# wvu-irl/flope

Hardware: AMD Instinct MI355X
Metric: poses_per_sec (higher is better)
Workload: dtype f16; 1 GPU; PoseResNet (ResNet-18 trunk + fp32 head) forward + special Procrustes + pose assembly, batch 256 x 224x224x3 16-bit NHWC crops resident in HBM per GPU (BASELINE configs[1]); one RCCL all-gather of the poses per run when N>1 (configs[3]); batch_per_gpu=256, global_batch=256, crop=224, parallelism=dp1, weights=synthetic_state_dict(seed 0), eval-mode BN folded

## Files before the change

### flope_amd/csrc/engine.hip

```cpp
#include "../../include/flope_amd.h"
#include "common.h"
#include "host_pack.h"

#include <math.h>
#include <stdio.h>
#include <stdlib.h>
#include <string.h>

#include <map>
#include <string>
#include <vector>

extern "C" int flope_conv_mfma_init();
extern "C" int flope_conv_mfma_launch(const ConvP* p, int dtype, int cfg, int patch, int nbuf, size_t lds, void* stream);
extern "C" int flope_stem_init();
extern "C" int flope_stem_launch(const StemP* p, int dtype, size_t lds, void* stream);
extern "C" int flope_maxpool_launch(const PoolP* p, int dtype, void* stream);
extern "C" int flope_avgpool_launch(const void* in, float* out, int B, int h, int w, int C, int dtype, void* stream);
extern "C" int flope_fc1_launch(const float* feat, const float* W1, const float* W1p, const float* b1, float* hidden, int B, int K, int N, void* stream);
extern "C" int flope_fc2_procrustes_launch(const float* hidden, const float* W2, const float* b2, float* r9, float* R, int B, int K, const float* xyz, int nullify, float* Rt, void* stream);
extern "C" int flope_fc2_procrustes_k4_launch(const float* hidden, const float* W2, const float* b2, float* r9, float* R, int B, int K, const float* xyz, int nullify, float* Rt, void* stream);
extern "C" int flope_prep_input_launch(const void* x, int in_format, int B, int H, int W, void* out, int Hip, int Wip, int dtype, void* stream);
extern "C" int flope_read_stage_launch(const void* in, float* out, int B, int C, int h, int w, int dtype, void* stream);
extern "C" int flope_naive_conv_launch(const NaiveConvP* p, void* stream);
extern "C" int flope_conv_stag_init();
extern "C" int flope_conv_gstag_init();
extern "C" int flope_conv_w4_init();
extern "C" int flope_conv_r4_init();
extern "C" int flope_conv_r4_ok(const ConvP* p);
extern "C" int flope_conv_r4_launch(const ConvP* p, int dtype, int grid_blocks, void* stream);
extern "C" int flope_conv_s1r_init();
extern "C" int flope_conv_s1r_ok(const ConvP* p);
extern "C" int flope_conv_s1r_launch(const ConvP* p, const void* w, int dtype, int grid, void* stream);
extern "C" int flope_conv_s2r_init();
extern "C" int flope_conv_s2r_ok(const ConvP* p);
extern "C" int flope_conv_s2r_launch(const ConvP* p, const void* w, int dtype, int grid, void* stream);
extern "C" int flope_conv_w4_launch(const ConvP* p, int dtype, int grid_blocks, int mt, void* stream);
extern "C" size_t flope_conv_w4_lds(int pt, int mt, int dsf, int pers);
extern "C" int flope_conv_gstag_launch(const ConvP* p, int dtype, void* stream);
extern "C" int flope_conv_stag_launch(const ConvP* p, int dtype, int grid_blocks, size_t lds, void* stream);
extern "C" int flope_conv_split_finalize_launch(const ConvP* p, int dtype, void* stream);
extern "C" int flope_stem_pool_init();
extern "C" int flope_stem_pool_r_blocks_per_cu();
#ifdef FLOPE_STAG_DBG
extern "C" void flope_stem_pool_set_dbg(void* ptr);
#endif
// ... 12 lines not shown
constexpr size_t kDbgRegion = 1 << 20;
constexpr size_t kBufSlack = 1 << 20;

struct Conv {
  std::string name, bn;
  int cin = 0, cout = 0, k = 0, stride = 1;
  int in_buf = -1, out_buf = -1, res_buf = -1;
  int hin = 0, win = 0, hout = 0, wout = 0;
  int relu = 0;
  int cfg = 0, patch = 0, nbuf = 2, per_image = 0, tiles_per_image = 0, mtiles = 0, ntiles = 0, rows_max = 0;
  size_t lds = 0;
  void* w_packed = nullptr;
  void* w_stag = nullptr;
  void* w_s2r = nullptr;
  void* w_s1r = nullptr;
  int stag = 0, stag_patch_bytes = 0, nseg = 1; size_t stag_lds = 0;
  int w4_patch[9] = {0};
  float* w_naive = nullptr;
  float* bias = nullptr;
  int folded = 0, ds_conv = -1;
  void* w_ds_stag = nullptr;
  void* w_ds_s1r = nullptr;
  float* bias_fused = nullptr;
  mutable std::string last_kernel, last_detail;
};

struct Buf { void* ptr = nullptr; size_t bytes = 0; int C = 0, h = 0, w = 0; };

}

struct flope_engine {
  int device = 0, H = 0, W = 0, maxB = 0, dtype = 0, bod = 2048;
  int esz = 2;
  int sHip = 0, sWip = 0, Hs = 0, Ws = 0, stem_tiles = 0, stem_rows = 0;
  size_t stem_lds = 0;
  void* stem_in = nullptr; size_t stem_in_bytes = 0;
  int* stem_q = nullptr;
  void* stem_w = nullptr; void* stem_w2 = nullptr; float* stem_w_naive = nullptr; float* stem_bias = nullptr;
  std::vector<Buf> bufs;
  std::vector<Conv> convs;
  int stage_buf[10];
  int final_buf = -1;
  float *feat = nullptr, *hidden = nullptr, *W1 = nullptr, *W1p = nullptr, *b1 = nullptr, *W2 = nullptr, *b2 = nullptr;
  float* r9_scratch = nullptr;
  bool weights_loaded = false;
  int opt_patch = 1, opt_bm256 = 1, opt_profile = 0, opt_nbuf = 2, opt_dbg = 0, opt_ldspad = 0, opt_fuse_stem = 1, opt_streams = 2, opt_persist = 0, num_cus = 256, opt_stag = 3, cur_slices = 1, plan_slices = 1, cur_batch = 1, opt_rows_grid = 0, opt_split = 0, opt_dsfuse = 1, opt_ksplit = 1, opt_fc1_packed = 1, opt_gstag = 1, opt_rowseg = 1, opt_stem_persist = 1, opt_skew = 1, opt_reslds = 1, opt_prio = 0, opt_r4 = 1, opt_w4cw = 4, opt_w4cwf = 0, opt_fc2_k4 = 1, opt_w4mt = 0, opt_w4mtlo = 0, opt_lag = 20, opt_w4 = 1, opt_stem_r = 1, opt_s2r = 1, opt_s2r_grid = 0, opt_s1r = 1;
  float* split_ws = nullptr; size_t split_ws_bytes = 0;
  hipStream_t side[4] = {nullptr, nullptr, nullptr, nullptr};
  hipEvent_t ev_fork = nullptr, ev_join[4] = {nullptr, nullptr, nullptr, nullptr};
  std::vector<hipEvent_t> ev;
  int ev_n = 0;
  std::vector<int> ev_slice;
  int mark_slice = 0;
  int last_batch = 0;
  bool last_fused = false;
  std::string err;
};

namespace {

int fail(flope_engine* e, int code, const std::string& msg) {
// ... 218 lines not shown
extern "C" const char* flope_version(void) { return "flope_amd 0.1 (gfx950; mfma_f32_16x16x32 bf16/f16; fp32 head)"; }

extern "C" int flope_engine_geometry(flope_handle h, int* max_batch, int* dtype, int* height, int* width, int* device_id) {
  if (!h) return FLOPE_EINVAL;
  if (max_batch) *max_batch = h->maxB;
  if (dtype) *dtype = h->dtype;
  if (height) *height = h->H;
  if (width) *width = h->W;
  if (device_id) *device_id = h->device;
  return FLOPE_OK;
}

extern "C" const char* flope_last_error(flope_handle h) { return h ? h->err.c_str() : g_last_error.c_str(); }

static int rebuild_plan(flope_engine* e) {
  for (Conv& c : e->convs) { plan_conv(e, c); c.folded = 0; c.ds_conv = -1; }
  if (e->opt_dsfuse && e->dtype != FLOPE_DT_F32)
    for (size_t i = 0; i + 1 < e->convs.size(); ++i) {
      Conv& cd = e->convs[i];
      Conv& c2 = e->convs[i + 1];
      if (cd.k == 1 && c2.k == 3 && c2.res_buf == cd.out_buf && c2.stag == 1 && c2.cout >= 128 && c2.stag_patch_bytes >= 4 &&
          c2.stag_patch_bytes != 7 && cd.cin % 64 == 0 && cd.stride == 2) {
        cd.folded = 1;
        c2.ds_conv = (int)i;
      }
    }
  return 0;
}

extern "C" int flope_create(int device_id, int height, int width, int max_batch, int dtype, int backbone_out_dim,
                            flope_handle* out) {
// ... 24 lines not shown
  {
    hipDeviceProp_t prop;
    CREATE_TRY(hipGetDeviceProperties(&prop, device_id));
    e->num_cus = prop.multiProcessorCount > 0 ? prop.multiProcessorCount : 256;
  }
  if (dtype != FLOPE_DT_F32) {
    int s = flope_conv_mfma_init();
    if (s == 0) s = flope_stem_init();
    if (s == 0) s = flope_stem_pool_init();
    if (s == 0) s = flope_conv_stag_init();
    if (s == 0) s = flope_conv_gstag_init();
    if (s == 0) s = flope_conv_w4_init();
    if (s == 0) s = flope_conv_r4_init();
    if (s == 0) s = flope_conv_s2r_init();
    if (s == 0) s = flope_conv_s1r_init();
    if (s != 0) { int rc = fail(nullptr, FLOPE_EHIP, std::string("kernel attribute setup: ") + hipGetErrorString((hipError_t)s)); flope_destroy(e); return rc; }
  }
  const size_t B = (size_t)max_batch;
  e->sHip = height + 6; e->sWip = (width + 8 + 1) & ~1;
  e->Hs = out_dim(height, 7, 2, 3); e->Ws = out_dim(width, 7, 2, 3);
  e->stem_in_bytes = B * e->sHip * e->sWip * 4 * e->esz;
  CREATE_TRY(hipMalloc(&e->stem_in, e->stem_in_bytes));
  CREATE_TRY(hipMemset(e->stem_in, 0, e->stem_in_bytes));
  {
    const int HoWo = e->Hs * e->Ws;
    e->stem_tiles = (HoWo + 255) / 256;
    int span = 1;
    for (int t = 0; t < e->stem_tiles; ++t) {
      const int m0 = t * 256, me = std::min(m0 + 256, HoWo);
      span = std::max(span, (me - 1) / e->Ws - m0 / e->Ws + 1);
// ... 62 lines not shown
  e->ev.resize(4 * (e->convs.size() + 8) + 2);
  e->ev_slice.assign(e->ev.size(), 0);
  for (hipEvent_t& ev : e->ev) CREATE_TRY(hipEventCreate(&ev));
  CREATE_TRY(hipDeviceSynchronize());
#undef CREATE_TRY
  rebuild_plan(e);
  *out = e;
  return FLOPE_OK;
}

extern "C" int flope_destroy(flope_handle e) {
  if (!e) return FLOPE_OK;
  hipSetDevice(e->device);
  hipDeviceSynchronize();
  for (Buf& b : e->bufs) if (b.ptr) hipFree(b.ptr);
  for (Conv& c : e->convs) { if (c.w_packed) hipFree(c.w_packed); if (c.w_stag) hipFree(c.w_stag); if (c.w_s2r) hipFree(c.w_s2r); if (c.w_s1r) hipFree(c.w_s1r); if (c.w_naive) hipFree(c.w_naive); if (c.bias) hipFree(c.bias); if (c.w_ds_stag) hipFree(c.w_ds_stag); if (c.w_ds_s1r) hipFree(c.w_ds_s1r); if (c.bias_fused) hipFree(c.bias_fused); }
  void* singles[] = {e->stem_in, e->stem_q, e->stem_w, e->stem_w2, e->stem_w_naive, e->stem_bias, e->feat, e->hidden, e->W1, e->W1p, e->b1, e->W2, e->b2, e->r9_scratch, e->split_ws};
  for (void* p : singles) if (p) hipFree(p);
  for (hipEvent_t ev : e->ev) hipEventDestroy(ev);
  for (int i = 0; i < 4; ++i) { if (e->side[i]) hipStreamDestroy(e->side[i]); if (e->ev_join[i]) hipEventDestroy(e->ev_join[i]); }
  if (e->ev_fork) hipEventDestroy(e->ev_fork);
  delete e;
  return FLOPE_OK;
}

extern "C" int flope_debug_read_ws(flope_handle e, void* dst_host, size_t offset, size_t bytes) {
  if (!e || !dst_host) return fail(e, FLOPE_EINVAL, "flope_debug_read_ws: NULL argument");
  if (!e->split_ws || offset + bytes > e->split_ws_bytes) return fail(e, FLOPE_EINVAL, "flope_debug_read_ws: out of range");
  HIP_TRY(e, hipSetDevice(e->device));
  HIP_TRY(e, hipDeviceSynchronize());
  HIP_TRY(e, hipMemcpy(dst_host, (const char*)e->split_ws + offset, bytes, hipMemcpyDeviceToHost));
// ... 6 lines not shown
  if (!strcmp(name, "patch")) { prev = e->opt_patch; e->opt_patch = value != 0; }
  else if (!strcmp(name, "bm256")) { prev = e->opt_bm256; e->opt_bm256 = value != 0; }
  else if (!strcmp(name, "persist")) { prev = e->opt_persist; e->opt_persist = value != 0; return prev; }
  else if (!strcmp(name, "rows_grid")) { prev = e->opt_rows_grid; e->opt_rows_grid = value < 0 ? -1 : value; return prev; }
  else if (!strcmp(name, "split")) { prev = e->opt_split; e->opt_split = value < 0 ? 0 : value; return prev; }
  else if (!strcmp(name, "fc1_packed")) { prev = e->opt_fc1_packed; e->opt_fc1_packed = value != 0; return prev; }
  else if (!strcmp(name, "w4mtlo")) { prev = e->opt_w4mtlo; e->opt_w4mtlo = value <= 0 ? 0 : (value < 5 ? 5 : (value > 8 ? 8 : value)); return prev; }
  else if (!strcmp(name, "lag")) { prev = e->opt_lag; e->opt_lag = value < 0 ? 0 : (value > 500 ? 500 : value); return prev; }
  else if (!strcmp(name, "w4mt")) { prev = e->opt_w4mt; e->opt_w4mt = (value >= 5 && value <= 8) ? value : 0; return prev; }
  else if (!strcmp(name, "fc2_k4")) { prev = e->opt_fc2_k4; e->opt_fc2_k4 = value != 0; return prev; }
  else if (!strcmp(name, "ksplit")) { prev = e->opt_ksplit; e->opt_ksplit = value < 0 ? 0 : (value > 2 ? 2 : value); return prev; }
  else if (!strcmp(name, "stem_r")) { prev = e->opt_stem_r; e->opt_stem_r = value != 0; return prev; }
  else if (!strcmp(name, "stem_persist")) { prev = e->opt_stem_persist; e->opt_stem_persist = value < 0 ? 0 : (value > 2 ? 2 : value); return prev; }
  else if (!strcmp(name, "rowseg")) { prev = e->opt_rowseg; e->opt_rowseg = value != 0; }
  else if (!strcmp(name, "skew")) { prev = e->opt_skew; e->opt_skew = value != 0; }
  else if (!strcmp(name, "r4")) { prev = e->opt_r4; e->opt_r4 = value != 0; return prev; }
  else if (!strcmp(name, "s1r")) { prev = e->opt_s1r; e->opt_s1r = value != 0; return prev; }
  else if (!strcmp(name, "s2r_grid")) { prev = e->opt_s2r_grid; e->opt_s2r_grid = value; return prev; }
  else if (!strcmp(name, "s2r")) { prev = e->opt_s2r; e->opt_s2r = value != 0; return prev; }
  else if (!strcmp(name, "w4")) { prev = e->opt_w4; e->opt_w4 = value != 0; return prev; }
  else if (!strcmp(name, "w4cw")) { prev = e->opt_w4cw; e->opt_w4cw = value < 0 ? 0 : (value > 64 ? 64 : value); return prev; }
  else if (!strcmp(name, "w4cwf")) { prev = e->opt_w4cwf; e->opt_w4cwf = value & 3; return prev; }
  else if (!strcmp(name, "prio")) { prev = e->opt_prio; e->opt_prio = value < 0 ? 0 : (value > 2 ? 2 : value); return prev; }
  else if (!strcmp(name, "reslds")) { prev = e->opt_reslds; e->opt_reslds = value != 0; return prev; }
  else if (!strcmp(name, "gstag")) { prev = e->opt_gstag; e->opt_gstag = value < 0 ? 0 : (value > 2 ? 2 : value); }
  else if (!strcmp(name, "dsfuse")) { prev = e->opt_dsfuse; e->opt_dsfuse = value != 0; }
  else if (!strcmp(name, "stag")) { prev = e->opt_stag; e->opt_stag = value < 0 ? 0 : (value > 3 ? 3 : value); }
  else if (!strcmp(name, "streams")) { prev = e->opt_streams; e->opt_streams = value < 1 ? 1 : (value > 4 ? 4 : value); return prev; }
  else if (!strcmp(name, "fuse_stem")) { prev = e->opt_fuse_stem; e->opt_fuse_stem = value != 0; return prev; }
  else if (!strcmp(name, "ldspad")) { prev = e->opt_ldspad; e->opt_ldspad = value; return prev; }
  else if (!strcmp(name, "dbg")) { prev = e->opt_dbg; e->opt_dbg = value; return prev; }
// ... 24 lines not shown
  if ((rc = fold(e, ts, "base.conv1", "base.bn1", 64, 3, 7, &wf, &bf)) != 0) return rc;
  if ((rc = upload(e, bf, (void**)&e->stem_bias)) != 0) return rc;
  if (e->dtype == FLOPE_DT_F32) { if ((rc = upload(e, naive_layout(wf, 64, 3, 7), (void**)&e->stem_w_naive)) != 0) return rc; }
  else {
    if ((rc = upload(e, pack_stem(wf, e->dtype), &e->stem_w)) != 0) return rc;
    if ((rc = upload(e, pack_stem_frag(wf, e->dtype), &e->stem_w2)) != 0) return rc;
  }
  for (Conv& c : e->convs) {
    if ((rc = fold(e, ts, c.name, c.bn, c.cout, c.cin, c.k, &wf, &bf)) != 0) return rc;
    if ((rc = upload(e, bf, (void**)&c.bias)) != 0) return rc;
    if (e->dtype == FLOPE_DT_F32) { if ((rc = upload(e, naive_layout(wf, c.cout, c.cin, c.k), (void**)&c.w_naive)) != 0) return rc; }
    else {
      if ((rc = upload(e, pack_conv(wf, c.cout, c.cin, c.k, e->dtype), &c.w_packed)) != 0) return rc;
      if (c.k == 3 && c.cin % 64 == 0 && (rc = upload(e, pack_conv32(wf, c.cout, c.cin, e->dtype), &c.w_stag)) != 0) return rc;
      if (c.k == 3 && c.stride == 1 && c.cin == 128 && c.cout == 128 && (rc = upload(e, pack_s1r(wf, c.cin, e->dtype), &c.w_s1r)) != 0) return rc;
      if (c.k == 3 && c.stride == 2 && c.cin == 64 && c.cout == 128 && (rc = upload(e, pack_s2r(wf, c.cout, c.cin, e->dtype), &c.w_s2r)) != 0) return rc;
      if (c.k == 1 && c.stride == 2 && c.cin == 64 && c.cout == 128 && (rc = upload(e, pack_s1r_ds(wf, c.cin, e->dtype), &c.w_ds_s1r)) != 0) return rc;
      if (c.k == 1 && c.cout >= 128 && c.cin % 64 == 0 && (rc = upload(e, pack_conv32_1x1(wf, c.cout, c.cin, e->dtype), &c.w_ds_stag)) != 0) return rc;
    }
    host_bias.push_back(bf);
  }
  for (size_t i = 0; i + 1 < e->convs.size(); ++i)
    if (e->convs[i].k == 1 && e->convs[i + 1].res_buf == e->convs[i].out_buf) {
      std::vector<float> sum = host_bias[i + 1];
      for (size_t j = 0; j < sum.size(); ++j) sum[j] += host_bias[i][j];
      if ((rc = upload(e, sum, (void**)&e->convs[i + 1].bias_fused)) != 0) return rc;
    }
  const float* w1 = ts.get(e, "base.fc.0.weight", {e->bod, 512}, &rc); if (!w1) return rc;
  const float* b1 = ts.get(e, "base.fc.0.bias", {e->bod}, &rc); if (!b1) return rc;
  const float* w2 = ts.get(e, "fc_rot.weight", {9, e->bod}, &rc); if (!w2) return rc;
// ... 58 lines not shown
      K_TRY(e, "stem (fp32)", flope_naive_conv_launch(&p, stream));
    } else {
      StemP p; memset(&p, 0, sizeof(p));
      p.in = stem_in; p.out = bs.ptr; p.w = e->stem_w; p.bias = e->stem_bias;
      p.B = batch; p.Hip = e->sHip; p.Wip = e->sWip; p.Ho = e->Hs; p.Wo = e->Ws;
      p.tiles_per_image = e->stem_tiles; p.patch_rows_max = e->stem_rows;
      SMARK();
      K_TRY(e, "stem", flope_stem_launch(&p, dt, e->stem_lds, stream));
    }
    PoolP pp; pp.in = bs.ptr; pp.out = bp.ptr; pp.B = batch; pp.Hip = bs.h + 2; pp.Wip = bs.w + 2; pp.C = 64; pp.Ho = bp.h; pp.Wo = bp.w;
    SMARK();
    K_TRY(e, "maxpool", flope_maxpool_launch(&pp, dt, stream));
  }
  for (const Conv& c : e->convs) {
    if (c.folded) continue;
    if (dt == FLOPE_DT_F32) {
      NaiveConvP p; memset(&p, 0, sizeof(p));
      p.in = (const float*)vb[c.in_buf].ptr; p.out = (float*)vb[c.out_buf].ptr;
      p.res = c.res_buf >= 0 ? (const float*)vb[c.res_buf].ptr : nullptr;
      p.w = c.w_naive; p.bias = c.bias;
      p.B = batch; p.Hip = c.hin + 2; p.Wip = c.win + 2; p.Cin_stored = c.cin; p.Cin = c.cin; p.Ho = c.hout; p.Wo = c.wout;
      p.Hop = c.hout + 2; p.Wop = c.wout + 2; p.Cout = c.cout; p.KH = c.k; p.KW = c.k; p.stride = c.stride;
      p.in_off = c.k == 3 ? 0 : 1; p.relu = c.relu;
      SMARK();
      K_TRY(e, c.name.c_str(), flope_naive_conv_launch(&p, stream));
    } else if (c.stag == 3) {
      ConvP p; conv_params(e, vb, c, batch, &p);
      p.w = c.w_stag; p.per_image = 0; p.mtiles = (p.M + 255) / 256; p.ntiles = c.cout / 128; p.total_tiles = p.mtiles * p.ntiles;
      SMARK();
      c.last_kernel = "conv_gstag_kernel<256x128,s2>"; c.last_detail.clear();
// ... 250 lines not shown
}

extern "C" double flope_forward_flops(flope_handle e, int batch) {
  if (!e) return 0.0;
  double macs = (double)e->Hs * e->Ws * 64 * 147;
  for (const Conv& c : e->convs) macs += (double)c.hout * c.wout * c.cout * c.cin * c.k * c.k;
  macs += 512.0 * e->bod + 9.0 * e->bod;
  return 2.0 * macs * batch;
}

static int head_launches(const flope_engine* e) { return (e->opt_fuse_stem && e->dtype != FLOPE_DT_F32) ? 1 : 3; }
static int tail_launches(const flope_engine*) { return 3; }
extern "C" int flope_forward_launches(flope_handle e) {
  if (!e) return 0;
  int n = (int)e->convs.size() + tail_launches(e) + head_launches(e);
  for (const Conv& c : e->convs) n -= c.folded;
  return n;
}

extern "C" int flope_profile_read(flope_handle e, float* ms_out, int cap) {
  if (!e || !ms_out) return fail(e, FLOPE_EINVAL, "flope_profile_read: NULL argument");
  if (e->opt_profile != 1 || e->ev_n < 2) return fail(e, FLOPE_ESTATE, "flope_profile_read: no forward with option profile = 1 (profile = 2 records a time line: flope_profile_timeline)");
  HIP_TRY(e, hipEventSynchronize(e->ev[e->ev_n - 1]));
  const int n = std::min(cap, e->ev_n - 1);
  for (int i = 0; i < n; ++i) HIP_TRY(e, hipEventElapsedTime(&ms_out[i], e->ev[i], e->ev[i + 1]));
  return n;
}

extern "C" int flope_profile_timeline(flope_handle e, float* ms_out, int* slice_out, int cap) {
  if (!e || !ms_out || !slice_out) return fail(e, FLOPE_EINVAL, "flope_profile_timeline: NULL argument");
  if (e->opt_profile != 2 || e->ev_n < 2) return fail(e, FLOPE_ESTATE, "flope_profile_timeline: no forward with option profile = 2");
  HIP_TRY(e, hipSetDevice(e->device));
  HIP_TRY(e, hipDeviceSynchronize());
  const int n = std::min(cap, e->ev_n);
  for (int i = 0; i < n; ++i) {
    ms_out[i] = 0.f;
    if (i > 0) HIP_TRY(e, hipEventElapsedTime(&ms_out[i], e->ev[0], e->ev[i]));
    slice_out[i] = e->ev_slice[i];
  }
  return n;
}

extern "C" int flope_launch_info(flope_handle e, int idx, int batch, char* name, int name_cap, double* flops) {
  if (!e || !name || name_cap < 1 || !flops) return fail(e, FLOPE_EINVAL, "flope_launch_info: NULL argument");
  std::vector<int> live;
  for (size_t i = 0; i < e->convs.size(); ++i) if (!e->convs[i].folded) live.push_back((int)i);
  const int nc = (int)live.size();
  const int nh = head_launches(e);
  if (idx < 0 || idx >= nc + tail_launches(e) + nh) return fail(e, FLOPE_EINVAL, "flope_launch_info: bad index");
  const bool f32 = e->dtype == FLOPE_DT_F32;
  std::string s; double f = 0.0;
  if (nh == 1) {
    if (idx == 0) { s = "input+stem+maxpool|stem_pool_kernel"; f = 2.0 * e->Hs * e->Ws * 64 * 147; }
  } else {
    if (idx == 0) s = "prep_input|prep_input_kernel";
    else if (idx == 1) { s = f32 ? "stem|naive_conv_kernel" : "stem|stem_mfma_kernel"; f = 2.0 * e->Hs * e->Ws * 64 * 147; }
    else if (idx == 2) s = "maxpool|maxpool_kernel";
  }
  idx += 3 - nh;
  if (idx < 3) {  }
  else if (idx < 3 + nc) {
    const Conv& c = e->convs[live[idx - 3]];
    int BM, BN; tile_dims(c.cfg, &BM, &BN);
    char k[96];
    if (f32) snprintf(k, sizeof k, "naive_conv_kernel");
    else if (c.stag == 3) snprintf(k, sizeof k, "conv_gstag_kernel<256x128,s2>");
    else if (e->opt_s1r && c.w_s1r && (c.ds_conv < 0 || e->convs[c.ds_conv].w_ds_s1r) && c.stag == 1 && c.wout == 28 && c.hout % 4 == 0) snprintf(k, sizeof k, "conv_s1r_kernel<4rows x28>");
    else if (w4_eligible(e, c)) snprintf(k, sizeof k, "conv_w4_kernel<256x128>");
    else if (c.stag == 2 && e->opt_r4 && c.nseg <= 1 && c.cin == 64 && c.cout == 64 && c.wout == 56 && c.hout % 8 == 0) snprintf(k, sizeof k, "conv_r4_kernel<8rows x56>");
    else if (c.stag) snprintf(k, sizeof k, c.stag == 2 ? "conv_stag_kernel<8rows x64>" : (c.cout == 64 ? "conv_stag_kernel<512x64>" : "conv_stag_kernel<256x128>"));
    else if (e->opt_s2r && c.w_s2r && c.wout == 28 && c.hout % 4 == 0) snprintf(k, sizeof k, "conv_s2r_kernel<4rows x28>");
    else snprintf(k, sizeof k, "conv_mfma_kernel<%dx%d,%s,ring%d>", BM, BN, c.patch ? "patch" : "gather", c.nbuf);
    if (!f32 && e->last_batch > 0 && !c.last_kernel.empty()) snprintf(k, sizeof k, "%s", c.last_kernel.c_str());
    s = c.name + ((!f32 && e->last_batch > 0) ? c.last_detail : std::string()) + "|" + k;
    f = 2.0 * c.hout * c.wout * c.cout * c.cin * c.k * c.k;
    if (c.ds_conv >= 0) {
      const Conv& cd = e->convs[c.ds_conv];
      s = c.name + "+shortcut" + ((!f32 && e->last_batch > 0) ? c.last_detail : std::string()) + "|" + k;
      f += 2.0 * cd.hout * cd.wout * cd.cout * cd.cin;
    }
  } else if (idx == 3 + nc) s = "avgpool|avgpool_kernel";
  else if (idx == 4 + nc) { s = "fc1|fc1_kernel"; f = 2.0 * 512 * e->bod; }
  else { s = "fc_rot+procrustes|fc2_procrustes_kernel"; f = 2.0 * 9 * e->bod; }
  snprintf(name, name_cap, "%s", s.c_str());
  *flops = f * batch;
  return FLOPE_OK;
}

extern "C" int flope_describe_plan(flope_handle e, char* buf, int buflen) {
  if (!e || !buf || buflen < 1) return FLOPE_EINVAL;
  std::string s;
  char line[256];
  snprintf(line, sizeof line, "stem: tiles/img=%d rows=%d lds=%zu\n", e->stem_tiles, e->stem_rows, e->stem_lds);
  s += line;
  for (const Conv& c : e->convs) {
    if (c.stag == 3) { snprintf(line, sizeof line, "%s: 3x3 s2 %d->%d out %dx%d conv_gstag 256x128 (gathered tiles) lds=147456\n", c.name.c_str(), c.cin, c.cout, c.hout, c.wout); s += line; continue; }
    if (c.folded) { snprintf(line, sizeof line, "%s: 1x1 s2 %d->%d out %dx%d folded into the next conv (conv_stag DSF)\n", c.name.c_str(), c.cin, c.cout, c.hout, c.wout); s += line; continue; }
    if (c.stag && c.ds_conv >= 0) { snprintf(line, sizeof line, "%s: 3x3 s1 %d->%d out %dx%d %s 256x128 patch_rounds=%d lds=%zu, shortcut folded in (+%d K)\n", c.name.c_str(), c.cin, c.cout, c.hout, c.wout, w4_eligible(e, c) ? "conv_w4" : "conv_stag", c.stag_patch_bytes, c.stag_lds, e->convs[c.ds_conv].cin); s += line; continue; }
    if (c.stag == 2 && c.nseg > 1) { snprintf(line, sizeof line, "%s: 3x3 s1 %d->%d out %dx%d conv_stag 8-row bands x %d column segments of 64 patch_rounds=%d lds=%zu\n", c.name.c_str(), c.cin, c.cout, c.hout, c.wout, c.nseg, c.stag_patch_bytes, c.stag_lds); s += line; continue; }
    if (c.stag == 1 && w4_eligible(e, c)) { snprintf(line, sizeof line, "%s: 3x3 s1 %d->%d out %dx%d conv_w4 256x128 patch_rounds=%d lds=%zu\n", c.name.c_str(), c.cin, c.cout, c.hout, c.wout, c.stag_patch_bytes, flope_conv_w4_lds(c.stag_patch_bytes, 8, 0, 0)); s += line; continue; }
    if (c.stag) { snprintf(line, sizeof line, c.stag == 2 ? "%s: 3x3 s1 %d->%d out %dx%d conv_stag 8-row bands x 64 patch_rounds=%d lds=%zu\n" : "%s: 3x3 s1 %d->%d out %dx%d conv_stag 256x128 patch_rounds=%d lds=%zu\n", c.name.c_str(), c.cin, c.cout, c.hout, c.wout, c.stag_patch_bytes, c.stag_lds); s += line; continue; }
    snprintf(line, sizeof line, "%s: %dx%d s%d %d->%d out %dx%d cfg=%d patch=%d ring=%d per_image=%d rows=%d lds=%zu\n", c.name.c_str(),
             c.k, c.k, c.stride, c.cin, c.cout, c.hout, c.wout, c.cfg, c.patch, c.nbuf, c.per_image, c.rows_max, c.lds);
    s += line;
  }
  snprintf(buf, buflen, "%s", s.c_str());
  return FLOPE_OK;
}
```

### flope_amd/csrc/host_pack.h

```cpp
#pragma once
#include <stdint.h>
#include <string.h>
#include <vector>

#define FLOPE_DT_BF16_ 0

namespace flope_host {

inline void fastdiv_magic(unsigned d, unsigned* mg, unsigned* sh) {
  unsigned l = 0;
  while ((1ull << l) < d) ++l;
  const unsigned long long num = 1ull << (31 + l);
  *mg = (unsigned)((num + d - 1) / d);
  *sh = 31 + l;
}

inline uint16_t f32_to_bf16(float f) {
  uint32_t u; memcpy(&u, &f, 4);
  if ((u & 0x7fffffffu) > 0x7f800000u) return (uint16_t)((u >> 16) | 0x0040u);
  u += 0x7fffu + ((u >> 16) & 1u);
  return (uint16_t)(u >> 16);
}

inline uint16_t f32_to_f16(float f) {
// ... 152 lines not shown
}

inline std::vector<uint16_t> pack_s1r_ds(const std::vector<float>& wf, int cin, int dtype) {
  std::vector<uint16_t> out((size_t)4 * 2 * 2 * 64 * 8);
  for (int cg = 0; cg < 4; ++cg)
    for (int kh = 0; kh < 2; ++kh)
      for (int ct = 0; ct < 2; ++ct)
        for (int lane = 0; lane < 64; ++lane)
          for (int j = 0; j < 8; ++j) {
            const int i = lane & 15, co = 32 * cg + 8 * (i >> 2) + 4 * ct + (i & 3), ci = 32 * kh + 8 * (lane >> 4) + j;
            out[((((size_t)cg * 2 + kh) * 2 + ct) * 64 + lane) * 8 + j] = cvt16(wf[(size_t)co * cin + ci], dtype);
          }
  return out;
}

inline std::vector<float> naive_layout(const std::vector<float>& wf, int cout, int cin, int k) {
  std::vector<float> out((size_t)cout * cin * k * k);
  for (int co = 0; co < cout; ++co)
    for (int ci = 0; ci < cin; ++ci)
      for (int ky = 0; ky < k; ++ky)
        for (int kx = 0; kx < k; ++kx)
          out[(((size_t)ky * k + kx) * cin + ci) * cout + co] = wf[(((size_t)co * cin + ci) * k + ky) * k + kx];
  return out;
}


inline std::vector<float> pack_fc1(const float* W1, int N, int K) {
  std::vector<float> out((size_t)N * K);
  const int KB = K / 32;
  for (int t = 0; t < N / 16; ++t)
// ... 11 lines not shown
```

Baseline: 262,700 poses/s.

## Fuse layer1 basic-block conv pairs into one kernel with LDS intermediate

Adds a conv_l1f kernel that runs both 3x3 64->64 convolutions of a layer1 basic block in one launch. Producer waves compute conv1 rows into an LDS ring while consumer waves compute conv2 plus the residual from the staged input. Each image is split into row-pair segments chosen by a cost heuristic. This removes the HBM round trip of the intermediate activation and one launch per block, in exchange for more LDS, a single block per CU, and halo recomputation at segment edges.

```diff
diff --git a/flope_amd/csrc/conv_l1f.hip b/flope_amd/csrc/conv_l1f.hip
--- /dev/null
+++ b/flope_amd/csrc/conv_l1f.hip
@@ -0,0 +1,281 @@
+#include "common.h"
+#include <type_traits>
+
+namespace {
+
+#pragma clang diagnostic push
+#pragma clang diagnostic ignored "-Winline-asm"
+__device__ __forceinline__ void l1f_glds16(const char* gptr, unsigned lds_addr) {
+  asm volatile("s_mov_b32 m0, %1\n\ts_nop 0\n\tglobal_load_lds_dwordx4 %0, off" ::"v"(gptr), "s"(lds_addr) : "memory", "m0");
+}
+#pragma clang diagnostic pop
+
+__device__ __forceinline__ int l1f_tile_px(int c) { return c < 4 ? 2 * c : (c < 12 ? 2 * (c - 4) + 1 : 2 * (c - 8)); }
+
+constexpr int kWo = 56, kPairs = 28, kRowB = 64 * 64, kNin = 10, kNim = 8, kStep = 18;
+constexpr int kInPlane = kNin * kRowB;
+constexpr int kImOff = 2 * kInPlane;
+constexpr int kImPlane = kNim * kRowB;
+constexpr int kLds = kImOff + 2 * kImPlane;
+
+struct L1fP {
+  const void* in;
+  void* out;
+  const float* bias1;
+  const float* bias2;
+  int B, Hip, Wip;
+  int nseg;
+  int relu1, relu2;
+};
+
+#define L1F_BARRIER()                                                                                          \
+  do {                                                                                                         \
+    __builtin_amdgcn_sched_barrier(0);                                                                         \
+    asm volatile("" ::: "memory");                                                                             \
+    __builtin_amdgcn_s_barrier();                                                                              \
+    asm volatile("" ::: "memory");                                                                             \
+    __builtin_amdgcn_sched_barrier(0);                                                                         \
+  } while (0)
+
+template <typename T, int ROLE, int P0, int NP>
+__device__ __forceinline__ void l1f_walk(const L1fP& p, const u32x4* __restrict__ wpk, char* smem, int wave, int lane) {
+  typedef typename Elem<T>::frag frag;
+  const int tid = wave * 64 + lane, g = lane >> 4, r16 = lane & 15, cg = wave & 1;
+  const int pcol = l1f_tile_px(r16);
+  const bool t3row = pcol >= 8;
+  int cst[9];
+#pragma unroll
+  for (int t = 0; t < 9; ++t) {
+    const int dy = t / 3, c = pcol + t % 3;
+    cst[t] = c * 64 + ((g ^ ((2 * (dy & 1) + (c >> 2)) & 3)) << 4);
+  }
+
+  const u32x4* const wl = wpk + (size_t)cg * kStep * 2 * 64 + lane;
+  frag wres[kStep][2];
+  f32x4 b4[2];
+#pragma unroll
+  for (int s = 0; s < kStep; ++s)
+#pragma unroll
+    for (int ct = 0; ct < 2; ++ct) wres[s][ct] = __builtin_bit_cast(frag, wl[(s * 2 + ct) * 64]);
+  const float* const bias = ROLE ? p.bias2 : p.bias1;
+#pragma unroll
+  for (int ct = 0; ct < 2; ++ct) b4[ct] = *(const f32x4*)(bias + 32 * cg + 8 * g + 4 * ct);
+
+  const int drow = wave & 1, dplane = (wave >> 1) & 1;
+  int dsrc[4];
+#pragma unroll
+  for (int j = 0; j < 4; ++j) {
+    const int px = 16 * j + (lane >> 2);
+    dsrc[j] = (drow * p.Wip + min(px, p.Wip - 1)) * 128 + dplane * 64 + (((lane & 3) ^ ((2 * drow + (px >> 2)) & 3)) << 4);
+  }
+  auto dma_pair = [&](int img, int rp) {
+    const char* const src = (const char*)p.in + ((size_t)img * p.Hip + rp) * p.Wip * 128;
+    const unsigned dst = (unsigned)(dplane * kInPlane + ((rp % kNin) + drow) * kRowB);
+#pragma unroll
+    for (int j = 0; j < 4; ++j)
+      l1f_glds16(src + dsrc[j], (unsigned)__builtin_amdgcn_readfirstlane((int)(dst + j * 1024 + (unsigned)(size_t)(__attribute__((address_space(3))) char*)smem)));
+  };
+
+#pragma unroll
+  for (int i = 0; i < 2 * kImPlane / (512 * 16); ++i) *(u32x4*)(smem + kImOff + (i * 512 + tid) * 16) = u32x4{0u, 0u, 0u, 0u};
+#pragma unroll
+  for (int s = 0; s < kStep; ++s)
+#pragma unroll
+    for (int ct = 0; ct < 2; ++ct) asm volatile("" : "+v"(wres[s][ct]));
+#pragma unroll
+  for (int ct = 0; ct < 2; ++ct) asm volatile("" : "+v"(b4[ct]));
+
+  int ooff[NP];
+#pragma unroll
+  for (int i = 0; i < NP; ++i) {
+    const int k = (P0 + i) * 16 + pcol, row = k >= kWo ? 1 : 0, col = k - row * kWo;
+    ooff[i] = ((row * p.Wip + col + 1) * 64 + 32 * cg + 8 * g) * 2;
+  }
+
+  auto vbase = [&](const int (&sb)[4], const int (&v3)[3], int grp, int t) -> int {
+    const int dy = t / 3;
+    int a = (grp == 0 ? sb[dy] : (grp == 1 ? v3[dy] : sb[dy + 1] + 512)) + cst[t];
+    asm volatile("" : "+v"(a));
+    return a;
+  };
+  auto tgrp = [](int pt) { return pt < 3 ? 0 : (pt == 3 ? 1 : 2); };
+  auto toff = [](int pt) { return pt < 3 ? pt * 1024 : (pt == 3 ? 0 : (pt - 4) * 1024); };
+  constexpr bool kG0 = P0 == 0, kG1 = P0 == 0 && NP == 4, kG2 = P0 + NP > 4;
+  auto step_bases = [&](const int (&sb)[4], const int (&v3)[3], int t, int (&va)[3]) {
+    if (kG0) va[0] = vbase(sb, v3, 0, t);
+    if (kG1) va[1] = vbase(sb, v3, 1, t);
+    if (kG2) va[2] = vbase(sb, v3, 2, t);
+  };
+  auto faddr = [&](const int (&va)[3], int pt, int hc, int plane_b) -> char* { return smem + va[tgrp(pt)] + toff(pt) + hc * plane_b; };
+  auto ring = [&](int off, int n, int R, int (&sb)[4], int (&v3)[3]) {
+#pragma unroll
+    for (int lr = 0; lr < 4; ++lr) sb[lr] = off + ((R + lr) % n) * kRowB;
+#pragma unroll
+    for (int dy = 0; dy < 3; ++dy) v3[dy] = t3row ? sb[dy + 1] - 512 : sb[dy] + 3072;
+  };
+
+  const int G = gridDim.x, total = p.B * p.nseg, L = kPairs / p.nseg;
+  for (int item = blockIdx.x; item < total; item += G) {
+    const int img = item / p.nseg, s0 = (item - img * p.nseg) * L, s1 = s0 + L;
+    const int p0 = max(s0 - 1, 0), p1 = min(s1, kPairs - 1);
+    if (s0 == 0) {
+      *(u32x4*)(smem + kImOff + (tid >> 8) * kImPlane + (tid & 255) * 16) = u32x4{0u, 0u, 0u, 0u};
+    }
+    if constexpr (ROLE == 0) {
+      dma_pair(img, 2 * p0);
+      dma_pair(img, 2 * p0 + 2);
+      asm volatile("s_waitcnt vmcnt(0)" ::: "memory");
+    }
+    asm volatile("s_waitcnt lgkmcnt(0)" ::: "memory");
+    L1F_BARRIER();
+    for (int q = p0; q <= s1 + 1; ++q) {
+      int sb[4], v3[3];
+      if constexpr (ROLE == 0) {
+        if (q + 1 <= p1) dma_pair(img, 2 * q + 4);
+        int wb[4], w3[3];
+        ring(kImOff, kNim, 2 * q, wb, w3);
+        f32x4 acc[NP][2];
+        if (q <= p1) {
+          ring(0, kNin, 2 * q, sb, v3);
+          frag xf[2][NP];
+          int va[3] = {0, 0, 0};
+          step_bases(sb, v3, 0, va);
+#pragma unroll
+          for (int pt = 0; pt < NP; ++pt) xf[0][pt] = *(const frag*)faddr(va, P0 + pt, 0, kInPlane);
+          __builtin_amdgcn_sched_barrier(0);
+#pragma unroll
+          for (int s = 0; s < kStep; ++s) {
+            if (s + 1 < kStep) step_bases(sb, v3, (s + 1) % 9, va);
+#pragma unroll
+            for (int pt = 0; pt < NP; ++pt) {
+#pragma unroll
+              for (int ct = 0; ct < 2; ++ct) acc[pt][ct] = Elem<T>::mfma(wres[s][ct], xf[s & 1][pt], s == 0 ? b4[ct] : acc[pt][ct]);
+              if (s + 1 < kStep) xf[(s + 1) & 1][pt] = *(const frag*)faddr(va, P0 + pt, (s + 1) / 9, kInPlane);
+              __builtin_amdgcn_sched_group_barrier(0x008, 2, 0);
+              if (s + 1 < kStep) __builtin_amdgcn_sched_group_barrier(0x100, 1, 0);
+            }
+          }
+          __builtin_amdgcn_sched_barrier(0);
+        }
+        int wa[3] = {0, 0, 0};
+        step_bases(wb, w3, 4, wa);
+#pragma unroll
+        for (int pt = 0; pt < NP; ++pt) {
+          u32x4 o = {0u, 0u, 0u, 0u};
+          if (q <= p1) {
+#pragma unroll
+            for (int ct = 0; ct < 2; ++ct) {
+              o[2 * ct] = pk_out16<T>(pack2<T>(acc[pt][ct][0], acc[pt][ct][1]), p.relu1);
+              o[2 * ct + 1] = pk_out16<T>(pack2<T>(acc[pt][ct][2], acc[pt][ct][3]), p.relu1);
+            }
+          }
+          *(u32x4*)faddr(wa, P0 + pt, cg, kImPlane) = o;
+        }
+        asm volatile("s_waitcnt vmcnt(0)" ::: "memory");
+      } else {
+        const int s = q - 2;
+        if (s >= s0) {
+          int rb[4], r3[3];
+          ring(kImOff, kNim, 2 * s, sb, v3);
+          ring(0, kNin, 2 * s, rb, r3);
+          f32x4 acc[NP][2];
+          frag xf[2][NP];
+          u32x4 rq[NP];
+          int va[3] = {0, 0, 0};
+          step_bases(sb, v3, 0, va);
+#pragma unroll
+          for (int pt = 0; pt < NP; ++pt) xf[0][pt] = *(const frag*)faddr(va, P0 + pt, 0, kImPlane);
+          __builtin_amdgcn_sched_barrier(0);
+#pragma unroll
+          for (int s_ = 0; s_ < kStep; ++s_) {
+            if (s_ + 1 < kStep) step_bases(sb, v3, (s_ + 1) % 9, va);
+            else step_bases(rb, r3, 4, va);
+#pragma unroll
+            for (int pt = 0; pt < NP; ++pt) {
+#pragma unroll
+              for (int ct = 0; ct < 2; ++ct) acc[pt][ct] = Elem<T>::mfma(wres[s_][ct], xf[s_ & 1][pt], s_ == 0 ? b4[ct] : acc[pt][ct]);
+              if (s_ + 1 < kStep) xf[(s_ + 1) & 1][pt] = *(const frag*)faddr(va, P0 + pt, (s_ + 1) / 9, kImPlane);
+              if (s_ + 1 == kStep) rq[pt] = *(const u32x4*)faddr(va, P0 + pt, cg, kInPlane);
+              __builtin_amdgcn_sched_group_barrier(0x008, 2, 0);
+              __builtin_amdgcn_sched_group_barrier(0x100, 1, 0);
+            }
+          }
+          __builtin_amdgcn_sched_barrier(0);
+          char* const ob = (char*)p.out + (((size_t)img * p.Hip + 2 * s + 1) * p.Wip) * 128;
+#pragma unroll
+          for (int pt = 0; pt < NP; ++pt) {
+            u32x4 o;
+#pragma unroll
+            for (int ct = 0; ct < 2; ++ct) {
+              f32x4 v = acc[pt][ct];
+              v[0] += unpack_lo<T>(rq[pt][2 * ct]); v[1] += unpack_hi<T>(rq[pt][2 * ct]);
+              v[2] += unpack_lo<T>(rq[pt][2 * ct + 1]); v[3] += unpack_hi<T>(rq[pt][2 * ct + 1]);
+              o[2 * ct] = pk_out16<T>(pack2<T>(v[0], v[1]), p.relu2);
+              o[2 * ct + 1] = pk_out16<T>(pack2<T>(v[2], v[3]), p.relu2);
+            }
+            *(u32x4*)(ob + ooff[pt]) = o;
+          }
+        }
+      }
+      asm volatile("s_waitcnt lgkmcnt(0)" ::: "memory");
+      L1F_BARRIER();
+    }
+  }
+  asm volatile("s_waitcnt vmcnt(0)" ::: "memory");
+}
+
+template <typename T>
+__global__ __launch_bounds__(512, 1) void conv_l1f_kernel(const L1fP p, const u32x4* __restrict__ w1, const u32x4* __restrict__ w2) {
+  extern __shared__ __attribute__((aligned(16))) char smem[];
+  const int lane = threadIdx.x & 63;
+  const int wave = __builtin_amdgcn_readfirstlane((int)(threadIdx.x >> 6));
+  const int half = (wave >> 1) & 1;
+  if (wave < 4) {
+    if (half == 0) l1f_walk<T, 0, 0, 4>(p, w1, smem, wave, lane);
+    else l1f_walk<T, 0, 4, 3>(p, w1, smem, wave, lane);
+  } else {
+    if (half == 1) l1f_walk<T, 1, 0, 4>(p, w2, smem, wave, lane);
+    else l1f_walk<T, 1, 4, 3>(p, w2, smem, wave, lane);
+  }
+}
+
+}
+
+extern "C" int flope_conv_l1f_ok(int cin, int cout, int hout, int wout) { return cin == 64 && cout == 64 && hout == 56 && wout == 56; }
+
+extern "C" int flope_conv_l1f_lds() { return kLds; }
+
+extern "C" int flope_conv_l1f_init() {
+  hipError_t e = hipSuccess;
+#define A(T) if (e == hipSuccess) e = hipFuncSetAttribute((const void*)conv_l1f_kernel<T>, hipFuncAttributeMaxDynamicSharedMemorySize, kLds);
+  A(bf16_t) A(f16_t)
+#undef A
+  return (int)e;
+}
+
+extern "C" int flope_conv_l1f_nseg(int batch, int num_cus) {
+  static const int kSeg[5] = {1, 2, 4, 7, 14};
+  int best = 1;
+  long best_cost = -1;
+  for (int nseg : kSeg) {
+    const long items = (long)batch * nseg, rounds = (items + num_cus - 1) / num_cus;
+    const long cost = rounds * (kPairs / nseg + 2 + (nseg > 1 ? 1 : 0));
+    if (best_cost < 0 || cost < best_cost) { best_cost = cost; best = nseg; }
+  }
+  return best;
+}
+
+extern "C" int flope_conv_l1f_launch(const void* x, void* y, const void* w1, const float* bias1, int relu1, const void* w2,
+                                     const float* bias2, int relu2, int batch, int nseg, int grid, int dtype, void* stream) {
+  if (!x || !y || !w1 || !w2 || !bias1 || !bias2 || batch < 1 || nseg < 1 || kPairs % nseg) return (int)hipErrorInvalidValue;
+  L1fP p;
+  p.in = x; p.out = y; p.bias1 = bias1; p.bias2 = bias2;
+  p.B = batch; p.Hip = kWo + 2; p.Wip = kWo + 2; p.nseg = nseg; p.relu1 = relu1; p.relu2 = relu2;
+  const int total = batch * nseg;
+  if (grid > total) grid = total;
+  if (grid < 1) return (int)hipErrorInvalidValue;
+  hipStream_t st = (hipStream_t)stream;
+  if (dtype == 0) hipLaunchKernelGGL(conv_l1f_kernel<bf16_t>, dim3(grid), dim3(512), (size_t)kLds, st, p, (const u32x4*)w1, (const u32x4*)w2);
+  else hipLaunchKernelGGL(conv_l1f_kernel<f16_t>, dim3(grid), dim3(512), (size_t)kLds, st, p, (const u32x4*)w1, (const u32x4*)w2);
+  return (int)hipGetLastError();
+}
diff --git a/flope_amd/csrc/engine.hip b/flope_amd/csrc/engine.hip
--- a/flope_amd/csrc/engine.hip
+++ b/flope_amd/csrc/engine.hip
@@ -30,6 +30,11 @@
 extern "C" int flope_conv_r4_ok(const ConvP* p);
 extern "C" int flope_conv_r4_launch(const ConvP* p, int dtype, int grid_blocks, void* stream);
 extern "C" int flope_conv_s1r_init();
+extern "C" int flope_conv_l1f_init();
+extern "C" int flope_conv_l1f_ok(int cin, int cout, int hout, int wout);
+extern "C" int flope_conv_l1f_nseg(int batch, int num_cus);
+extern "C" int flope_conv_l1f_launch(const void* x, void* y, const void* w1, const float* bias1, int relu1, const void* w2,
+                                     const float* bias2, int relu2, int batch, int nseg, int grid, int dtype, void* stream);
 extern "C" int flope_conv_s1r_ok(const ConvP* p);
 extern "C" int flope_conv_s1r_launch(const ConvP* p, const void* w, int dtype, int grid, void* stream);
 extern "C" int flope_conv_s2r_init();
@@ -72,11 +77,13 @@
   void* w_stag = nullptr;
   void* w_s2r = nullptr;
   void* w_s1r = nullptr;
+  void* w_l1r = nullptr;
   int stag = 0, stag_patch_bytes = 0, nseg = 1; size_t stag_lds = 0;
   int w4_patch[9] = {0};
   float* w_naive = nullptr;
   float* bias = nullptr;
   int folded = 0, ds_conv = -1;
+  int carried = 0, l1f_conv1 = -1;
   void* w_ds_stag = nullptr;
   void* w_ds_s1r = nullptr;
   float* bias_fused = nullptr;
@@ -102,7 +109,7 @@
   float *feat = nullptr, *hidden = nullptr, *W1 = nullptr, *W1p = nullptr, *b1 = nullptr, *W2 = nullptr, *b2 = nullptr;
   float* r9_scratch = nullptr;
   bool weights_loaded = false;
-  int opt_patch = 1, opt_bm256 = 1, opt_profile = 0, opt_nbuf = 2, opt_dbg = 0, opt_ldspad = 0, opt_fuse_stem = 1, opt_streams = 2, opt_persist = 0, num_cus = 256, opt_stag = 3, cur_slices = 1, plan_slices = 1, cur_batch = 1, opt_rows_grid = 0, opt_split = 0, opt_dsfuse = 1, opt_ksplit = 1, opt_fc1_packed = 1, opt_gstag = 1, opt_rowseg = 1, opt_stem_persist = 1, opt_skew = 1, opt_reslds = 1, opt_prio = 0, opt_r4 = 1, opt_w4cw = 4, opt_w4cwf = 0, opt_fc2_k4 = 1, opt_w4mt = 0, opt_w4mtlo = 0, opt_lag = 20, opt_w4 = 1, opt_stem_r = 1, opt_s2r = 1, opt_s2r_grid = 0, opt_s1r = 1;
+  int opt_patch = 1, opt_bm256 = 1, opt_profile = 0, opt_nbuf = 2, opt_dbg = 0, opt_ldspad = 0, opt_fuse_stem = 1, opt_streams = 2, opt_persist = 0, num_cus = 256, opt_stag = 3, cur_slices = 1, plan_slices = 1, cur_batch = 1, opt_rows_grid = 0, opt_split = 0, opt_dsfuse = 1, opt_ksplit = 1, opt_fc1_packed = 1, opt_gstag = 1, opt_rowseg = 1, opt_stem_persist = 1, opt_skew = 1, opt_reslds = 1, opt_prio = 0, opt_r4 = 1, opt_w4cw = 4, opt_w4cwf = 0, opt_fc2_k4 = 1, opt_w4mt = 0, opt_w4mtlo = 0, opt_lag = 20, opt_w4 = 1, opt_stem_r = 1, opt_s2r = 1, opt_s2r_grid = 0, opt_s1r = 1, opt_l1f = 1;
   float* split_ws = nullptr; size_t split_ws_bytes = 0;
   hipStream_t side[4] = {nullptr, nullptr, nullptr, nullptr};
   hipEvent_t ev_fork = nullptr, ev_join[4] = {nullptr, nullptr, nullptr, nullptr};
@@ -351,7 +358,19 @@
 extern "C" const char* flope_last_error(flope_handle h) { return h ? h->err.c_str() : g_last_error.c_str(); }
 
 static int rebuild_plan(flope_engine* e) {
-  for (Conv& c : e->convs) { plan_conv(e, c); c.folded = 0; c.ds_conv = -1; }
+  for (Conv& c : e->convs) { plan_conv(e, c); c.folded = 0; c.ds_conv = -1; c.carried = 0; c.l1f_conv1 = -1; }
+  if (e->opt_l1f && e->opt_r4 && e->dtype != FLOPE_DT_F32)
+    for (size_t i = 0; i + 1 < e->convs.size(); ++i) {
+      Conv& c1 = e->convs[i];
+      Conv& c2 = e->convs[i + 1];
+      auto r4_shape = [](const Conv& c) {
+        return c.k == 3 && c.stride == 1 && c.stag == 2 && c.nseg <= 1 && flope_conv_l1f_ok(c.cin, c.cout, c.hout, c.wout);
+      };
+      if (r4_shape(c1) && r4_shape(c2) && c2.in_buf == c1.out_buf && c2.res_buf == c1.in_buf && c1.res_buf < 0 && !c1.carried) {
+        c1.carried = 1;
+        c2.l1f_conv1 = (int)i;
+      }
+    }
   if (e->opt_dsfuse && e->dtype != FLOPE_DT_F32)
     for (size_t i = 0; i + 1 < e->convs.size(); ++i) {
       Conv& cd = e->convs[i];
@@ -406,6 +425,7 @@
     if (s == 0) s = flope_conv_r4_init();
     if (s == 0) s = flope_conv_s2r_init();
     if (s == 0) s = flope_conv_s1r_init();
+    if (s == 0) s = flope_conv_l1f_init();
     if (s != 0) { int rc = fail(nullptr, FLOPE_EHIP, std::string("kernel attribute setup: ") + hipGetErrorString((hipError_t)s)); flope_destroy(e); return rc; }
   }
   const size_t B = (size_t)max_batch;
@@ -498,7 +518,7 @@
   hipSetDevice(e->device);
   hipDeviceSynchronize();
   for (Buf& b : e->bufs) if (b.ptr) hipFree(b.ptr);
-  for (Conv& c : e->convs) { if (c.w_packed) hipFree(c.w_packed); if (c.w_stag) hipFree(c.w_stag); if (c.w_s2r) hipFree(c.w_s2r); if (c.w_s1r) hipFree(c.w_s1r); if (c.w_naive) hipFree(c.w_naive); if (c.bias) hipFree(c.bias); if (c.w_ds_stag) hipFree(c.w_ds_stag); if (c.w_ds_s1r) hipFree(c.w_ds_s1r); if (c.bias_fused) hipFree(c.bias_fused); }
+  for (Conv& c : e->convs) { if (c.w_packed) hipFree(c.w_packed); if (c.w_stag) hipFree(c.w_stag); if (c.w_s2r) hipFree(c.w_s2r); if (c.w_s1r) hipFree(c.w_s1r); if (c.w_l1r) hipFree(c.w_l1r); if (c.w_naive) hipFree(c.w_naive); if (c.bias) hipFree(c.bias); if (c.w_ds_stag) hipFree(c.w_ds_stag); if (c.w_ds_s1r) hipFree(c.w_ds_s1r); if (c.bias_fused) hipFree(c.bias_fused); }
   void* singles[] = {e->stem_in, e->stem_q, e->stem_w, e->stem_w2, e->stem_w_naive, e->stem_bias, e->feat, e->hidden, e->W1, e->W1p, e->b1, e->W2, e->b2, e->r9_scratch, e->split_ws};
   for (void* p : singles) if (p) hipFree(p);
   for (hipEvent_t ev : e->ev) hipEventDestroy(ev);
@@ -535,7 +555,8 @@
   else if (!strcmp(name, "stem_persist")) { prev = e->opt_stem_persist; e->opt_stem_persist = value < 0 ? 0 : (value > 2 ? 2 : value); return prev; }
   else if (!strcmp(name, "rowseg")) { prev = e->opt_rowseg; e->opt_rowseg = value != 0; }
   else if (!strcmp(name, "skew")) { prev = e->opt_skew; e->opt_skew = value != 0; }
-  else if (!strcmp(name, "r4")) { prev = e->opt_r4; e->opt_r4 = value != 0; return prev; }
+  else if (!strcmp(name, "r4")) { prev = e->opt_r4; e->opt_r4 = value != 0; }
+  else if (!strcmp(name, "l1f")) { prev = e->opt_l1f; e->opt_l1f = value != 0; }
   else if (!strcmp(name, "s1r")) { prev = e->opt_s1r; e->opt_s1r = value != 0; return prev; }
   else if (!strcmp(name, "s2r_grid")) { prev = e->opt_s2r_grid; e->opt_s2r_grid = value; return prev; }
   else if (!strcmp(name, "s2r")) { prev = e->opt_s2r; e->opt_s2r = value != 0; return prev; }
@@ -590,6 +611,7 @@
       if ((rc = upload(e, pack_conv(wf, c.cout, c.cin, c.k, e->dtype), &c.w_packed)) != 0) return rc;
       if (c.k == 3 && c.cin % 64 == 0 && (rc = upload(e, pack_conv32(wf, c.cout, c.cin, e->dtype), &c.w_stag)) != 0) return rc;
       if (c.k == 3 && c.stride == 1 && c.cin == 128 && c.cout == 128 && (rc = upload(e, pack_s1r(wf, c.cin, e->dtype), &c.w_s1r)) != 0) return rc;
+      if (c.k == 3 && c.stride == 1 && c.cin == 64 && c.cout == 64 && (rc = upload(e, pack_l1r(wf, c.cin, e->dtype), &c.w_l1r)) != 0) return rc;
       if (c.k == 3 && c.stride == 2 && c.cin == 64 && c.cout == 128 && (rc = upload(e, pack_s2r(wf, c.cout, c.cin, e->dtype), &c.w_s2r)) != 0) return rc;
       if (c.k == 1 && c.stride == 2 && c.cin == 64 && c.cout == 128 && (rc = upload(e, pack_s1r_ds(wf, c.cin, e->dtype), &c.w_ds_s1r)) != 0) return rc;
       if (c.k == 1 && c.cout >= 128 && c.cin % 64 == 0 && (rc = upload(e, pack_conv32_1x1(wf, c.cout, c.cin, e->dtype), &c.w_ds_stag)) != 0) return rc;
@@ -678,6 +700,17 @@
   }
   for (const Conv& c : e->convs) {
     if (c.folded) continue;
+    if (c.carried && dt != FLOPE_DT_F32) continue;
+    if (c.l1f_conv1 >= 0 && dt != FLOPE_DT_F32) {
+      const Conv& c1 = e->convs[c.l1f_conv1];
+      if (!c1.w_l1r || !c.w_l1r) return fail(e, FLOPE_ESTATE, c.name + ": conv_l1f weight images missing");
+      const int nseg = flope_conv_l1f_nseg(e->cur_batch, e->num_cus);
+      SMARK();
+      c.last_kernel = "conv_l1f_kernel<2rows x56>"; c.last_detail.clear();
+      K_TRY(e, c.name.c_str(), flope_conv_l1f_launch(vb[c1.in_buf].ptr, vb[c.out_buf].ptr, c1.w_l1r, c1.bias, c1.relu, c.w_l1r, c.bias, c.relu,
+                                                     batch, nseg, e->num_cus, dt, stream));
+      continue;
+    }
     if (dt == FLOPE_DT_F32) {
       NaiveConvP p; memset(&p, 0, sizeof(p));
       p.in = (const float*)vb[c.in_buf].ptr; p.out = (float*)vb[c.out_buf].ptr;
@@ -958,7 +991,7 @@
 extern "C" int flope_forward_launches(flope_handle e) {
   if (!e) return 0;
   int n = (int)e->convs.size() + tail_launches(e) + head_launches(e);
-  for (const Conv& c : e->convs) n -= c.folded;
+  for (const Conv& c : e->convs) n -= c.folded + (e->dtype != FLOPE_DT_F32 ? c.carried : 0);
   return n;
 }
 
@@ -988,7 +1021,7 @@
 extern "C" int flope_launch_info(flope_handle e, int idx, int batch, char* name, int name_cap, double* flops) {
   if (!e || !name || name_cap < 1 || !flops) return fail(e, FLOPE_EINVAL, "flope_launch_info: NULL argument");
   std::vector<int> live;
-  for (size_t i = 0; i < e->convs.size(); ++i) if (!e->convs[i].folded) live.push_back((int)i);
+  for (size_t i = 0; i < e->convs.size(); ++i) if (!e->convs[i].folded && !(e->convs[i].carried && e->dtype != FLOPE_DT_F32)) live.push_back((int)i);
   const int nc = (int)live.size();
   const int nh = head_launches(e);
   if (idx < 0 || idx >= nc + tail_launches(e) + nh) return fail(e, FLOPE_EINVAL, "flope_launch_info: bad index");
@@ -1018,6 +1051,11 @@
     if (!f32 && e->last_batch > 0 && !c.last_kernel.empty()) snprintf(k, sizeof k, "%s", c.last_kernel.c_str());
     s = c.name + ((!f32 && e->last_batch > 0) ? c.last_detail : std::string()) + "|" + k;
     f = 2.0 * c.hout * c.wout * c.cout * c.cin * c.k * c.k;
+    if (c.l1f_conv1 >= 0 && !f32) {
+      const Conv& c1 = e->convs[c.l1f_conv1];
+      s = c1.name + "+conv2|conv_l1f_kernel<2rows x56>";
+      f += 2.0 * c1.hout * c1.wout * c1.cout * c1.cin * c1.k * c1.k;
+    }
     if (c.ds_conv >= 0) {
       const Conv& cd = e->convs[c.ds_conv];
       s = c.name + "+shortcut" + ((!f32 && e->last_batch > 0) ? c.last_detail : std::string()) + "|" + k;
@@ -1041,6 +1079,8 @@
     if (c.stag == 3) { snprintf(line, sizeof line, "%s: 3x3 s2 %d->%d out %dx%d conv_gstag 256x128 (gathered tiles) lds=147456\n", c.name.c_str(), c.cin, c.cout, c.hout, c.wout); s += line; continue; }
     if (c.folded) { snprintf(line, sizeof line, "%s: 1x1 s2 %d->%d out %dx%d folded into the next conv (conv_stag DSF)\n", c.name.c_str(), c.cin, c.cout, c.hout, c.wout); s += line; continue; }
     if (c.stag && c.ds_conv >= 0) { snprintf(line, sizeof line, "%s: 3x3 s1 %d->%d out %dx%d %s 256x128 patch_rounds=%d lds=%zu, shortcut folded in (+%d K)\n", c.name.c_str(), c.cin, c.cout, c.hout, c.wout, w4_eligible(e, c) ? "conv_w4" : "conv_stag", c.stag_patch_bytes, c.stag_lds, e->convs[c.ds_conv].cin); s += line; continue; }
+    if (c.carried) { snprintf(line, sizeof line, "%s: 3x3 s1 %d->%d out %dx%d carried by the next launch (conv_l1f: the block in one launch, the intermediate in LDS; 8-row bands of conv_r4 with l1f = 0)\n", c.name.c_str(), c.cin, c.cout, c.hout, c.wout); s += line; continue; }
+    if (c.l1f_conv1 >= 0) { snprintf(line, sizeof line, "%s: 3x3 s1 %d->%d out %dx%d conv_l1f row pairs with %s (8-row bands of conv_r4 with l1f = 0) lds=%d\n", c.name.c_str(), c.cin, c.cout, c.hout, c.wout, e->convs[c.l1f_conv1].name.c_str(), 147456); s += line; continue; }
     if (c.stag == 2 && c.nseg > 1) { snprintf(line, sizeof line, "%s: 3x3 s1 %d->%d out %dx%d conv_stag 8-row bands x %d column segments of 64 patch_rounds=%d lds=%zu\n", c.name.c_str(), c.cin, c.cout, c.hout, c.wout, c.nseg, c.stag_patch_bytes, c.stag_lds); s += line; continue; }
     if (c.stag == 1 && w4_eligible(e, c)) { snprintf(line, sizeof line, "%s: 3x3 s1 %d->%d out %dx%d conv_w4 256x128 patch_rounds=%d lds=%zu\n", c.name.c_str(), c.cin, c.cout, c.hout, c.wout, c.stag_patch_bytes, flope_conv_w4_lds(c.stag_patch_bytes, 8, 0, 0)); s += line; continue; }
     if (c.stag) { snprintf(line, sizeof line, c.stag == 2 ? "%s: 3x3 s1 %d->%d out %dx%d conv_stag 8-row bands x 64 patch_rounds=%d lds=%zu\n" : "%s: 3x3 s1 %d->%d out %dx%d conv_stag 256x128 patch_rounds=%d lds=%zu\n", c.name.c_str(), c.cin, c.cout, c.hout, c.wout, c.stag_patch_bytes, c.stag_lds); s += line; continue; }
diff --git a/flope_amd/csrc/host_pack.h b/flope_amd/csrc/host_pack.h
--- a/flope_amd/csrc/host_pack.h
+++ b/flope_amd/csrc/host_pack.h
@@ -190,6 +190,20 @@
   return out;
 }
 
+inline std::vector<uint16_t> pack_l1r(const std::vector<float>& wf, int cin, int dtype) {
+  std::vector<uint16_t> out((size_t)2 * 18 * 2 * 64 * 8);
+  for (int cg = 0; cg < 2; ++cg)
+    for (int st = 0; st < 18; ++st)
+      for (int ct = 0; ct < 2; ++ct)
+        for (int lane = 0; lane < 64; ++lane)
+          for (int j = 0; j < 8; ++j) {
+            const int i = lane & 15, hc = st / 9, tap = st % 9, ky = tap / 3, kx = tap % 3;
+            const int co = 32 * cg + 8 * (i >> 2) + 4 * ct + (i & 3), ci = 32 * hc + 8 * (lane >> 4) + j;
+            out[((((size_t)cg * 18 + st) * 2 + ct) * 64 + lane) * 8 + j] = cvt16(wf[(((size_t)co * cin + ci) * 3 + ky) * 3 + kx], dtype);
+          }
+  return out;
+}
+
 inline std::vector<float> naive_layout(const std::vector<float>& wf, int cout, int cin, int k) {
   std::vector<float> out((size_t)cout * cin * k * k);
   for (int co = 0; co < cout; ++co)
```

Result: no change. 265,300 poses/s (median of 6 runs) (+1.0%).
